# Sartor02/libMultiRobotPlanning

Hardware: AMD Instinct MI355X
Metric: low_level_node_expansions_per_sec (higher is better)
Workload: dtype int32

## Files before the change

### libmultirobotplanning_amd/csrc/ll_compact.h

```cpp
#pragma once
#include <stddef.h>
#include <stdint.h>

namespace mrp {
namespace ct {

using namespace wv;

#ifndef WV_HAS_UNMASKED_GLOADS
WV_FN V gLoadU16(const uint16_t* base, V idx) { return gLoadU16m(base, idx, bsplat(true)); }
WV_FN V gLoad32(const uint32_t* base, V idx) { return gLoad32m(base, idx, bsplat(true)); }
#endif

constexpr uint32_t kRowBytes = 128;
constexpr uint32_t oCtl = 0;
constexpr uint32_t oJob = 256;
constexpr uint32_t oRes = 384;
constexpr uint32_t oOpen = 448;
constexpr uint32_t kFront = 0xFFFFFFFFu;
template <uint32_t GROUPS, uint32_t FH_BITS, uint32_t F_BITS, uint32_t L_BITS, bool LONGT = false>
struct TierCfg {
  static constexpr bool kLongT = LONGT;
  static constexpr uint32_t kGroups = GROUPS;
  static constexpr uint32_t kCap = 256u * GROUPS - 1u;
// ... 56 lines not shown
constexpr uint32_t windowBytes(bool bg) { return Narrow::windowBytes(bg); }
constexpr uint32_t kBitsBytes = Narrow::kBitsBytes, kParentBytes = Narrow::kParentBytes;
constexpr uint32_t kMO = Narrow::kMO, kMF = Narrow::kMF, kEmpty = Narrow::kEmpty, kMaxT = Narrow::kMaxT;
constexpr uint32_t kHeapClamp = Narrow::kHeapClamp;
static_assert(oOpen % 16 == 0, "LDS areas are 16-byte aligned");

enum : int32_t { C_OK = 0, C_NO_SOLUTION = 1, C_CAP_EXP = 2, C_OVERFLOW = -1 };

struct CJob {
  uint32_t dimx, dimy, sx, sy, gx, gy;
  int32_t lastGoal;
  float w;
  uint32_t nVc, nEc;
  uint32_t obstWords;
  uint32_t nAgentsPad, tPad;
  uint32_t maxExp;
  uint32_t openCap, maxT;
  uint32_t taNoGoal;
  uint32_t rows;
  uint64_t vc;
  uint64_t ec;
  uint64_t obst;
  uint64_t pathsG;
  uint64_t parentTab;
  uint64_t outPath;
  uint64_t bitsG;
};
static_assert(sizeof(CJob) <= oRes - oJob && sizeof(CJob) % 4 == 0, "CJob fits its block of the window");
struct CRes {
  int32_t status, cost, fmin, nStates;
  uint32_t expanded, nodes;
};
#ifdef MRP_CT_PROF
#define MRP_CT_PROF_DECL uint32_t prof_[8] = {0, 0, 0, 0, 0, 0, 0, 0}; uint64_t profT_ = wv::clock64()
#define MRP_CT_PROF_MARK(k) do { const uint64_t n_ = wv::clock64(); prof_[k] += (uint32_t)(n_ - profT_); profT_ = n_; } while (0)
#define MRP_CT_PROF_ADD(k, v) prof_[k] += (v)
#define MRP_CT_PROF_STORE(lds) do { for (uint32_t q_ = 0; q_ < 8; ++q_) ldsStoreS(lds, oRes + 32u + 4u * q_, prof_[q_]); } while (0)
#elif defined(MRP_CT_ASM_MARKS)
#define MRP_CT_PROF_DECL do { } while (0)
#define MRP_CT_PROF_MARK(k) asm volatile("; PHASE " #k ::: "memory")
#define MRP_CT_PROF_ADD(k, v) do { } while (0)
#define MRP_CT_PROF_STORE(lds) do { } while (0)
#else
#define MRP_CT_PROF_DECL do { } while (0)
#define MRP_CT_PROF_MARK(k) do { } while (0)
#define MRP_CT_PROF_ADD(k, v) do { } while (0)
#define MRP_CT_PROF_STORE(lds) do { } while (0)
#endif
static_assert(sizeof(CRes) <= 32 && oRes + 64 <= oOpen, "CRes fits its block of the window");

#ifndef MRP_CT_COUNT
#define MRP_CT_COUNT(k, v) do { } while (0)
#endif

#define MRP_CT_JOB_U32(lds, field) ldsLoadS(lds, oJob + (uint32_t)offsetof(CJob, field))
template <class T>
WV_FN T* jobPtr(Lds lds, uint32_t off) {
  const uint64_t lo = ldsLoadS(lds, oJob + off), hi = ldsLoadS(lds, oJob + off + 4u);
  return (T*)(uintptr_t)(lo | (hi << 32));
}
#define MRP_CT_JOB_PTR(T, lds, field) jobPtr<T>(lds, (uint32_t)offsetof(CJob, field))

WV_FN uint32_t popc64(uint64_t v) { return (uint32_t)__builtin_popcountll(v); }
WV_FN uint32_t ctz64(uint64_t v) { return (uint32_t)__builtin_ctzll(v); }
WV_FN uint32_t ctz32(uint32_t v) { return (uint32_t)__builtin_ctz(v); }
WV_FN uint32_t lg2(uint32_t v) { return 31u - (uint32_t)__builtin_clz(v); }
WV_FN uint32_t lo32(uint64_t v) { return (uint32_t)v; }
WV_FN uint32_t hi32(uint64_t v) { return (uint32_t)(v >> 32); }

#ifndef WV_HAS_MASK_SLICES
WV_FN V maskShr(uint64_t m, V sh) { return sel((sh & 32u) != 0u, splat(hi32(m)), splat(lo32(m))) >> (sh & 16u); }
WV_FN V bitSel(V pick, V a, V b) { return (a & pick) | (b & ~pick); }
WV_FN B lowLanes(uint32_t m) { return (((splat(m) >> laneId()) & 1u) != 0u) & (laneId() < 32u); }
#endif

struct Sides {
  V lane, l5;
  B isB;
  V lvl, off1;
  V anc, needR;
};
WV_FN Sides makeSides() {
  Sides s;
  s.lane = laneId();
  s.l5 = s.lane & 31u;
  s.isB = (s.lane >> 5) != 0u;
  const V n = s.l5 + 1u;
  s.lvl = 31u - clz(n);
  s.off1 = sel(s.l5 == 31u, splat(0x100000u), n - (splat(1u) << s.lvl) - 1u);
  s.anc = splat(0u);
  s.needR = splat(0u);
  for (uint32_t k = 1; k <= 4; ++k) {
    const V a = n >> k;
    const B has = (a != 0u) & (n < 32u);
    s.anc |= sel(has, splat(1u) << (a - 1u), splat(0u));
    s.needR |= sel(has, ((n >> (k - 1u)) & 1u) << (a - 1u), splat(0u));
  }
  return s;
}
WV_FN V bothSides(const Sides& S, uint32_t a, uint32_t b) { return sel(S.isB, splat(b), splat(a)); }

WV_FN V dualDescend(Lds lds, const Sides& S, V hb, V km, V cMax, V xk) {
  V idx = splat(0u);
  for (;;) {
    const V node = ((idx + 1u) << S.lvl) + S.off1;
    V c = node * 2u + 1u;
    c = sel(c < cMax, c, cMax);
    const V2 pr = ldsLoad64(lds, hb + c * 4u);
    const V kl = pr.x & km, kr = pr.y & km;
    const B right = kl < kr;
    const V pe = sel(right, pr.y, pr.x);
    const V pk = sel(right, kr, kl);
    const B go = pk >= xk;
    const uint64_t goM = ballot(go), rM = ballot(right);
    const V g32 = bothSides(S, lo32(goM), hi32(goM));
    const V r32 = bothSides(S, lo32(rM), hi32(rM));
    const B reached = ((g32 & S.anc) == S.anc) & (((r32 ^ S.needR) & S.anc) == 0u);
    const B onPath = reached & go;
    const uint64_t pM = ballot(onPath);
    ldsStore32m(lds, hb + node * 4u, pe, onPath);
    const V pm = bothSides(S, lo32(pM), hi32(pM));
    const V steps = popc(pm);
    const V d = 31u - clz(pm | 1u);
    const V rel = d * 2u + 1u + ((r32 >> d) & 1u);
    idx = sel(pm != 0u, ((idx + 1u) << steps) + rel - (splat(1u) << steps), idx);
    if (ballot(steps == 5u) == 0ull) break;
  }
  return idx;
}

WV_FN void dualSiftUp(Lds lds, const Sides& S, V hb, V km, V p1, uint32_t e, bool idleA, bool idleB) {
  const V ancPos = (p1 >> (S.l5 + 1u)) - 1u;
  const V ae = ldsLoad32(lds, hb + ancPos * 4u);
  const uint64_t worse = ballot((ae & km) < (km & e));
  const uint32_t stopA = idleA ? 0u : ctz32(~lo32(worse)) + 1u, stopB = idleB ? 0u : ctz32(~hi32(worse)) + 1u;
  const V stop1 = bothSides(S, stopA, stopB);
  const V dest = (p1 >> S.l5) - 1u;
  ldsStore32m(lds, hb + dest * 4u, sel((S.l5 + 1u) == stop1, splat(e), ae), S.l5 < stop1);
}

struct Rows {
  V l4;
  B isY, isSecond;
};
WV_FN Rows makeRows() {
  Rows r;
  const V lane = laneId();
  r.l4 = lane & 15u;
  r.isY = (lane >> 5) != 0u;
  r.isSecond = ((lane >> 4) & 1u) != 0u;
  return r;
}
WV_FN V perRow(const Rows& R, uint32_t x1, uint32_t x2, uint32_t y1, uint32_t y2) {
  return sel(R.isY, sel(R.isSecond, splat(y2), splat(y1)), sel(R.isSecond, splat(x2), splat(x1)));
}

WV_FN void pushPairs(Lds lds, const Rows& R, uint32_t hbX, uint32_t kmX, uint32_t pX, uint32_t nX, uint32_t eX1, uint32_t eX2,
                     uint32_t hbY, uint32_t kmY, uint32_t pY, uint32_t nY, uint32_t eY1, uint32_t eY2) {
  const V hb = sel(R.isY, splat(hbY), splat(hbX));
  const V km = sel(R.isY, splat(kmY), splat(kmX));
  const V p1 = perRow(R, nX >= 1u ? pX + 1u : 1u, nX >= 2u ? pX + 2u : 1u, nY >= 1u ? pY + 1u : 1u, nY >= 2u ? pY + 2u : 1u);
  const V e = perRow(R, eX1, eX2, eY1, eY2);
  const V ek = e & km;
  const V ancIdx = p1 >> (R.l4 + 1u);
  const V ae = ldsLoad32(lds, hb + ancIdx * 4u - 4u);
  const V dest = hb + (p1 >> R.l4) * 4u - 4u;
  const uint64_t worse1 = ballot((ae & km) < ek);
  const uint32_t sX1 = nX >= 1u ? ctz32(~lo32(worse1)) + 1u : 0u, sY1 = nY >= 1u ? ctz32(~hi32(worse1)) + 1u : 0u;
  const V stop1 = sel(R.isY, splat(sY1), splat(sX1));
  ldsStore32m(lds, dest, sel((R.l4 + 1u) == stop1, e, ae), (!R.isSecond) & (R.l4 < stop1));
  if (nX >= 2u || nY >= 2u) {
#ifndef MRP_CT_PLAIN_EXPANSION
    const uint32_t ddX = ((pX + 2u) & (pX + 1u)) == 0u ? 1u : 0u, ddY = ((pY + 2u) & (pY + 1u)) == 0u ? 1u : 0u;
#else
    const uint32_t ddX = lg2(pX + 2u) - lg2(pX + 1u), ddY = lg2(pY + 2u) - lg2(pY + 1u);
#endif
    const V dd = sel(R.isY, splat(ddY), splat(ddX));
    const V e1 = sel(R.isY, splat(eY1), splat(eX1));
    const V j1p1 = R.l4 + 1u - dd;
    const B shared = (R.l4 >= dd) & (ancIdx == ((p1 - 1u) >> j1p1));
    const V up = rowShl1(ae, kFront);
    const V now = sel(shared, sel((j1p1 + 1u) < stop1, up, sel((j1p1 + 1u) == stop1, e1, ae)), sel((p1 == 2u) & (R.l4 == 0u), e1, ae));
    const uint64_t worse2 = ballot((now & km) < ek);
    const uint32_t sX2 = nX >= 2u ? ctz32(~(lo32(worse2) >> 16)) + 1u : 0u, sY2 = nY >= 2u ? ctz32(~(hi32(worse2) >> 16)) + 1u : 0u;
    const V stop2 = sel(R.isY, splat(sY2), splat(sX2));
    ldsStore32m(lds, dest, sel((R.l4 + 1u) == stop2, e, now), R.isSecond & (R.l4 < stop2));
  }
}

template <bool EPS, bool PLDS, bool BG = false, class C = Narrow>
WV_ENTRY int32_t compactSearch(Lds window) {
  constexpr uint32_t kGroups = C::kGroups, kHeapClamp = C::kHeapClamp, kAuxCap = C::kAuxCap, kAuxBytes = C::kAuxBytes,
                     kAuxClamp = C::kAuxClamp, kRows = C::kRows, kBitsBytes = C::kBitsBytes;
  constexpr uint32_t oFocal = C::oFocal, oAux = C::oAux, oBits = C::oBits;
  constexpr uint32_t kMO = C::kMO, kMF = C::kMF, kEmpty = C::kEmpty, kMOAux = C::kMOAux, kAuxShift = C::kAuxShift;
  constexpr uint32_t kFShift = C::kFShift, kFhShift = C::kFhShift, kFMax = C::kFMax, kFhMax = C::kFhMax, kGMax = C::kGMax;
  constexpr uint32_t oObstX = C::obstOff(BG), oPathsX = C::pathsOff(BG);
  constexpr uint32_t oBuild = BG ? oOpen : oBits;
  const Lds lds = windowBase(window);
  const Sides S = makeSides();
  const Rows Rw = makeRows();
  const V lane = S.lane;
  const V hb = bothSides(S, oOpen + 4u, oFocal + 4u);
  const V km = bothSides(S, kMO, kMF);
  const V hbAux = splat(oAux + 4u), kmAux = splat(kMOAux);
  const uint32_t dimx = MRP_CT_JOB_U32(lds, dimx), dimy = MRP_CT_JOB_U32(lds, dimy);
  const uint32_t gx = MRP_CT_JOB_U32(lds, gx), gy = MRP_CT_JOB_U32(lds, gy);
  const uint32_t nEc = MRP_CT_JOB_U32(lds, nEc);
  const uint32_t nAgentsPad = EPS ? MRP_CT_JOB_U32(lds, nAgentsPad) : 0u;
  int32_t status = C_NO_SOLUTION, cost = 0, fmin = 0, nStates = 0;
  uint32_t nOpen = 1, nFocal = EPS ? 1u : 0u, nodes = 1, expansions = 0;

  MRP_CT_PROF_DECL;
  sync();
  uint32_t* bitsG = BG ? MRP_CT_JOB_PTR(uint32_t, lds, bitsG) : nullptr;
  {
    const uint32_t* obst = MRP_CT_JOB_PTR(const uint32_t, lds, obst);
    const uint32_t obstWords = MRP_CT_JOB_U32(lds, obstWords);
    const V y = S.l5;
    const V bitOff = y * dimx;
    const V wi = bitOff >> 5, sh = bitOff & 31u;
    const B rowIn = (y < dimy) & !S.isB;
    const V lo = gLoad32m(obst, wi, rowIn & (wi < obstWords));
    const V hi = gLoad32m(obst, wi + 1u, rowIn & ((wi + 1u) < obstWords));
    V w = sel(sh == 0u, lo, (lo >> sh) | (hi << (splat(32u) - sh)));
    const uint32_t colMask = dimx >= 32u ? 0xFFFFFFFFu : ((1u << dimx) - 1u);
    w = (w & colMask) | ~colMask;
    w = sel(rowIn, w, splat(0xFFFFFFFFu));
    ldsStore32m(lds, splat(oObstX) + y * 4u, w, !S.isB);
  }
  auto initHeaps = [&]() {
    const V4 none{splat(kEmpty), splat(kEmpty), splat(kEmpty), splat(kEmpty)};
    const V4 head{sel(lane == 0u, splat(kFront), splat(kEmpty)), splat(kEmpty), splat(kEmpty), splat(kEmpty)};
    ldsStore128(lds, splat(oOpen) + lane * 16u, head);
    ldsStore128(lds, splat(oFocal) + lane * 16u, head);
    ldsStore128(lds, splat(oAux) + lane * 16u, head);
    for (uint32_t g = 1; g < kGroups; ++g) {
      ldsStore128(lds, splat(oOpen + g * 1024u) + lane * 16u, none);
      ldsStore128(lds, splat(oFocal + g * 1024u) + lane * 16u, none);
    }
// ... 30 lines not shown
    const V4 head{sel(lane == 0u, splat(kFront), splat(kEmpty)), splat(kEmpty), splat(kEmpty), splat(kEmpty)};
    ldsStore128(lds, splat(oAux) + lane * 16u, head);
    for (uint32_t b = 1024u; b < kAuxBytes; b += 1024u) ldsStore128m(lds, splat(oAux + b) + lane * 16u, none, (lane * 16u + b) < kAuxBytes);
    sync();
    rowsReady += kRows;
  };
  if (C::kLongT) {
    moreRows();
  } else if (BG) {
    constexpr uint32_t kBuildRows = C::kBuildRows;
    for (uint32_t r0 = 0; r0 < kRows; r0 += kBuildRows) {
      buildRows(oBuild, r0, kBuildRows);
      sync();
      for (uint32_t i = 0; i < kBuildRows * kRowBytes / 1024u; ++i)
        gStore128(bitsG, splat(r0 * (kRowBytes / 16u) + i * 64u) + lane, ldsLoad128(lds, splat(oBuild + i * 1024u) + lane * 16u));
      sync();
    }
    initHeaps();
  } else {
    buildRows(oBuild, 0u, kRows);
  }
  V ecReg = splat(0xFFFFFFFFu);
  if (nEc) {
    const uint32_t* ec = MRP_CT_JOB_PTR(const uint32_t, lds, ec);
    ldsStore32(lds, splat(oAux + 16u) + lane * 4u, sel(lane < nEc, gLoad32m(ec, lane, lane < nEc), splat(0xFFFFFFFFu)));
    sync();
    ecReg = ldsLoad32(lds, splat(oAux + 16u) + lane * 4u);
    sync();
    const V4 none{splat(kEmpty), splat(kEmpty), splat(kEmpty), splat(kEmpty)};
    ldsStore128m(lds, splat(oAux + 16u) + lane * 16u, none, lane < 16u);
  }
  const V dx = sel(lane == 1u, splat(0xFFFFFFFFu), sel(lane == 2u, splat(1u), sel(lane < 5u, splat(0u), splat(0x4000u))));
  const V dy = sel(lane == 3u, splat(1u), sel(lane == 4u, splat(0xFFFFFFFFu), splat(0u)));
#ifndef MRP_CT_PLAIN_EXPANSION
  const bool grid = EPS && nAgentsPad != 0u && nAgentsPad <= 16u;
#else
  const bool grid = false;
#endif
  const V agent0 = grid ? Rw.l4 : lane;
  const B in0 = agent0 < nAgentsPad, in1 = (lane + 64u) < nAgentsPad;
  const V col0 = sel(in0, agent0, splat(nAgentsPad ? nAgentsPad - 1u : 0u));
  const V col1 = sel(in1, lane + 64u, splat(nAgentsPad ? nAgentsPad - 1u : 0u));
  const V gridD = perRow(Rw, 0xFFFFFFFFu, 1u, 256u, 0xFFFFFF00u);
  const V gridSh = ((lane - 1u) & 3u) << 4;
  const V gridWait = sel(lane == 0u, splat(0xFFFFFFFFu), splat(0u));
  const uint32_t tPad = EPS ? MRP_CT_JOB_U32(lds, tPad) : 0u;
  const uint16_t* pathsG = PLDS ? nullptr : MRP_CT_JOB_PTR(const uint16_t, lds, pathsG);
  const int32_t lastGoal = (int32_t)MRP_CT_JOB_U32(lds, lastGoal);
  const float wBound = uintAsFloat(MRP_CT_JOB_U32(lds, w));
  const uint32_t maxExp = MRP_CT_JOB_U32(lds, maxExp), openCap = MRP_CT_JOB_U32(lds, openCap), maxT = MRP_CT_JOB_U32(lds, maxT);
  uint8_t* parentTab = MRP_CT_JOB_PTR(uint8_t, lds, parentTab);
  const uint32_t goalCell = gx | (gy << 5);
  int32_t bestF;
  {
    const uint32_t sx = MRP_CT_JOB_U32(lds, sx), sy = MRP_CT_JOB_U32(lds, sy);
    const uint32_t h0 = (sx > gx ? sx - gx : gx - sx) + (sy > gy ? sy - gy : gy - sy);
    bestF = (int32_t)h0;
    const uint32_t e0 = (kFhMax << kFhShift) | ((kFMax - h0) << kFShift) | ((C::kLongT ? 63u - h0 : 0u) << 10) | (sx | (sy << 5));
    ldsStoreS(lds, oOpen + 4u, e0);
    if (EPS) ldsStoreS(lds, oFocal + 4u, e0);
  }
  sync();
  MRP_CT_PROF_MARK(0);

  for (;;) {
    if (nOpen == 0u) {
      status = C_NO_SOLUTION;
      break;
    }
    const V tops = ldsLoad32(lds, hb);
    const uint32_t topO = readlane(tops, 0);
    uint32_t curE = EPS ? readlane(tops, 32) : topO;
    if (EPS) {
      const int32_t fTop = (int32_t)(kFMax - ((topO >> kFShift) & kFMax));
      const int32_t oldBest = bestF;
      bestF = fTop;
      if (fTop > oldBest) {
        MRP_CT_PROF_MARK(0);
        const float lo = fmulRn((float)oldBest, wBound), hi = fmulRn((float)fTop, wBound);
        bool bandEmpty = false;
#ifndef MRP_CT_FORCE_WALK
        {
          const int32_t fA = (int32_t)lo + 1, fBraw = (int32_t)hi;
          const int32_t fB = fBraw > (int32_t)kFMax - 1 ? (int32_t)kFMax - 1 : fBraw;
          bandEmpty = true;
          if (fB >= fA) {
            const V base = splat(kFMax - (uint32_t)fB), span = splat((uint32_t)(fB - fA));
            for (uint32_t g = 0; g < kGroups && g * 256u <= nOpen; ++g) {
              const V4 grp = ldsLoad128(lds, splat(oOpen + g * 1024u) + lane * 16u);
              const B in = ((((grp.x >> kFShift) & kFMax) - base) <= span) | ((((grp.y >> kFShift) & kFMax) - base) <= span) |
                           ((((grp.z >> kFShift) & kFMax) - base) <= span) | ((((grp.w >> kFShift) & kFMax) - base) <= span);
              if (ballot(in)) {
                bandEmpty = false;
                break;
              }
            }
          }
        }
#endif
        MRP_CT_PROF_ADD(7, bandEmpty ? 1u : 0u);
        if (!bandEmpty) {
        uint32_t npq = 0, npqHigh = 0;
        uint32_t cur = 0, curKey = topO & kMO, eCur = topO;
        V trio = ldsLoad32(lds, splat(oOpen + 4u) + sel(lane == 2u, splat(cur), splat(2u * cur + 1u) + (lane & 1u)) * 4u);
        for (;;) {
          MRP_CT_PROF_ADD(6, 1u);
          const uint32_t firstC = 2u * cur + 1u;
          const uint32_t nCh = firstC + 1u < nOpen ? 2u : firstC < nOpen ? 1u : 0u;
          if (npq + 2u > kAuxCap) {
            status = C_OVERFLOW;
            cost = 4;
            break;
          }
          const uint32_t e1 = readlane(trio, 0), e2 = readlane(trio, 1);
          const float fv = (float)(int32_t)(kFMax - ((curKey >> kFShift) & kFMax));
          const bool inBand = fv > lo && fv <= hi;
          pushPairs(lds, Rw, oAux + 4u, kMOAux, npq, nCh, ((e1 & kMO) << kAuxShift) | firstC, ((e2 & kMO) << kAuxShift) | (firstC + 1u),
                    oFocal + 4u, kMF, nFocal,
                    inBand ? 1u : 0u, eCur, 0u);
          npq += nCh;
          nFocal += inBand ? 1u : 0u;
          npqHigh = npq > npqHigh ? npq : npqHigh;
          if (fv > hi) break;
          if (npq == 0u) break;
          npq -= 1u;
          const V two = ldsLoad32(lds, splat(oAux + 4u) + sel(lane == 0u, splat(0u), splat(npq)) * 4u);
          ldsStoreS(lds, oAux + 4u + 4u * npq, kEmpty);
          uint32_t hole = 0, above = kFront;
          bool first = true;
          uint32_t value = 0;
          for (;;) {
            const V node = ((splat(hole) + 1u) << S.lvl) + S.off1;
            V c = node * 2u + 1u;
            c = sel(c < kAuxClamp, c, splat(kAuxClamp));
            const V2 pr = ldsLoad64(lds, splat(oAux + 4u) + c * 4u);
            if (first) {
              first = false;
              const uint32_t curA = readlane(two, 0);
              value = readlane(two, 1);
              cur = curA & C::kAuxIdxMask;
              curKey = (curA >> kAuxShift) & kMO;
              trio = ldsLoad32(lds, splat(oOpen + 4u) + sel(lane == 2u, splat(cur), splat(2u * cur + 1u) + (lane & 1u)) * 4u);
              if (npq == 0u) break;
            }
            const V kl = pr.x & kMOAux, kr = pr.y & kMOAux;
            const B right = kr >= kl;
            const V pe = sel(right, pr.y, pr.x);
            const B go = kl > (kEmpty & kMOAux);
            const uint32_t goM = lo32(ballot(go)), rM = lo32(ballot(right));
            const B onPath = ((S.anc & goM) == S.anc) & (((S.needR ^ rM) & S.anc) == 0u) & go;
            const uint32_t pm = lo32(ballot(onPath & !S.isB));
            ldsStore32m(lds, splat(oAux + 4u) + node * 4u, pe, onPath);
            if (pm == 0u) break;
            const uint32_t steps = (uint32_t)__builtin_popcount(pm), d = lg2(pm);
            hole = ((hole + 1u) << steps) + 2u * d + 1u + ((rM >> d) & 1u) - (1u << steps);
            above = readlane(pe, d);
            if (steps < 5u) break;
          }
          eCur = readlane(trio, 2);
          if (npq > 0u) {
            if (hole == 0u || !((above & kMOAux) < (value & kMOAux)))
              ldsStoreS(lds, oAux + 4u + 4u * hole, value);
            else
              dualSiftUp(lds, S, hbAux, kmAux, splat(hole + 1u), value, false, false);
          }
        }
        for (uint32_t b = 0; b <= 4u * npqHigh; b += 1024u) {
          const V4 none{splat(kEmpty), splat(kEmpty), splat(kEmpty), splat(kEmpty)};
          const V4 head{sel(lane == 0u, splat(kFront), splat(kEmpty)), splat(kEmpty), splat(kEmpty), splat(kEmpty)};
          ldsStore128m(lds, splat(oAux + b) + lane * 16u, b == 0u ? head : none, (lane * 16u + b) < kAuxBytes);
        }
        if (status == C_OVERFLOW) break;
        curE = ldsLoadS(lds, oFocal + 4u);
        }
        MRP_CT_PROF_MARK(1);
      }
    }
    const uint32_t cell = curE & 1023u, curFh = kFhMax - (curE >> kFhShift);
    const uint32_t t = C::kLongT ? (kFMax - ((curE >> kFShift) & kFMax)) - (63u - ((curE >> 10) & 63u)) : (curE >> 10) & kGMax;
    const uint32_t x = cell & 31u, y = cell >> 5;
    const bool isGoal = cell == goalCell && (int32_t)t > lastGoal;
    if (!isGoal) {
      if (nOpen + 5u > openCap || t > maxT || (EPS && !C::kExactFhCheck && curFh + 2u * nAgentsPad > kFhMax)) {
        status = C_OVERFLOW;
        cost = nOpen + 5u > openCap ? 1 : t > maxT ? 2 : 3;
        break;
      }
    }
    expansions += 1u;
    if (expansions > maxExp) {
      status = C_CAP_EXP;
      break;
    }
    if (isGoal) {
      status = C_OK;
      cost = (int32_t)t;
      fmin = (int32_t)(kFMax - (((EPS ? topO : curE) >> kFShift) & kFMax));
      nStates = (int32_t)t + 1;
      uint16_t* outPath = MRP_CT_JOB_PTR(uint16_t, lds, outPath);
      sync();
      uint32_t c = cell;
      const uint32_t* tab32 = (const uint32_t*)parentTab;
      constexpr int32_t kStage = BG ? (int32_t)C::kStageRows : 8;
      for (int32_t k0 = (int32_t)t; k0 >= 1; k0 -= kStage) {
        V rowW[kStage][4];
        for (int32_t r = 0; r < kStage; ++r)
          for (uint32_t q = 0; q < 4; ++q)
            rowW[r][q] = (k0 - r >= 1) ? gLoad32Coherent(tab32, splat((uint32_t)(k0 - r) * 256u + q * 64u) + lane) : splat(0u);
        for (int32_t r = 0; r < kStage; ++r)
          for (uint32_t q = 0; q < 4; ++q) ldsStore32(lds, splat(oBuild + (uint32_t)r * 1024u + q * 256u) + lane * 4u, rowW[r][q]);
        sync();
        for (int32_t r = 0; r < kStage && k0 - r >= 1; ++r) {
          const uint32_t k = (uint32_t)(k0 - r);
          gStoreU16m(outPath, splat(k), splat((c & 31u) | ((c >> 5) << 8)), lane == 0u);
          const uint32_t a = first(ldsLoadU8(lds, splat(oBuild + (uint32_t)r * 1024u + c)));
          c = a == 1u ? c + 1u : a == 2u ? c - 1u : a == 3u ? c - 32u : a == 4u ? c + 32u : c;
        }
        sync();
      }
      gStoreU16m(outPath, splat(0u), splat((c & 31u) | ((c >> 5) << 8)), lane == 0u);
      break;
    }

    MRP_CT_PROF_MARK(0);
    const uint32_t t1 = t + 1u;
    if (C::kLongT && t1 >= rowsReady) moreRows();
// ... 21 lines not shown
          a1 = gLoadU16(pathsG, splat(ra * nAgentsPad) + col1);
          b1 = gLoadU16(pathsG, splat(rb * nAgentsPad) + col1);
        }
      }
    }

    MRP_CT_PROF_MARK(2);
    {
      const uint32_t nOld = nOpen;
      nOpen -= 1u;
      if (EPS) nFocal -= 1u;
      const V lastAddr = hb + bothSides(S, nOpen, nFocal) * 4u;
      const V lastV = ldsLoad32(lds, lastAddr);
      uint32_t p = 0;
#ifndef MRP_CT_PLAIN_EXPANSION
      const bool atRoot = EPS && ((curE ^ topO) & C::kStateMask) == 0u;
#else
      const bool atRoot = false;
#endif
      MRP_CT_COUNT(0, atRoot ? 1u : 0u);
      MRP_CT_COUNT(6, atRoot && nOld > 512u ? 1u : 0u);
      if (EPS && !atRoot) {
        const V key = splat(curE & C::kStateMask);
        for (uint32_t g = 0; g < kGroups && g * 256u <= nOld; ++g) {
          MRP_CT_COUNT(1, 1u);
          const V4 grp = ldsLoad128(lds, splat(oOpen + g * 1024u) + lane * 16u);
          const B m0 = (grp.x & C::kStateMask) == key, m1 = (grp.y & C::kStateMask) == key, m2 = (grp.z & C::kStateMask) == key,
                  m3 = (grp.w & C::kStateMask) == key;
          const uint64_t any = ballot(m0 | m1 | m2 | m3);
          if (any) {
            const V pos = lane * 4u + sel(m0, splat(0xFFFFFFFFu), sel(m1, splat(0u), sel(m2, splat(1u), splat(2u))));
            p = g * 256u + readlane(pos, ctz64(any));
            if (kGroups > 4u) break;
          }
        }
      }
      uint32_t lastO = readlane(lastV, 0);
      const uint32_t lastF = EPS ? readlane(lastV, 32) : kFront;
      ldsStore32m(lds, lastAddr, splat(kEmpty), S.l5 == 0u);
      if (EPS && !atRoot) {
        const uint32_t depth = lg2(p + 1u);
        MRP_CT_COUNT(4, p >= 256u ? 1u : 0u);
        MRP_CT_COUNT(5, p == nOld - 1u && depth != 0u ? 1u : 0u);
        const B act = !S.isB & (S.l5 < depth);
        const V ancPos = (splat(p + 1u) >> (S.l5 + 1u)) - 1u;
        const V ae = ldsLoad32(lds, splat(oOpen + 4u) + ancPos * 4u);
        ldsStore32m(lds, splat(oOpen + 4u) + ((splat(p + 1u) >> S.l5) - 1u) * 4u, ae, act);
        if (p == nOld - 1u && depth != 0u) {
          lastO = readlane(ae, 0);
          ldsStoreS(lds, oOpen + 4u + 4u * p, kEmpty);
        }
      }
      const V xk = bothSides(S, lastO & kMO, lastF & kMF);
      const V hole = dualDescend(lds, S, hb, km, splat(kHeapClamp), xk);
      ldsStore32m(lds, hb + hole * 4u, bothSides(S, lastO, lastF), (S.l5 == 0u) & (bothSides(S, nOpen, EPS ? nFocal : 0u) != 0u));
    }

    MRP_CT_PROF_MARK(3);
    const B okV = inb & (((word >> (nx & 31u)) & 1u) == 0u);
    uint32_t mask = lo32(ballot(okV)) & 0x1Fu;
    if (nEc) {
      const uint32_t base = (t << 19) | ((y * dimx + x) << 3);
      const V d = ecReg - base;
      if (ballot(d < 5u)) {
        uint32_t blocked = 0;
        for (uint32_t k = 0; k < 5u; ++k) blocked |= ballot(d == k) ? (1u << k) : 0u;
        mask &= ~blocked;
      }
    }
    if (mask == 0u) {
      MRP_CT_PROF_MARK(4);
      continue;
    }

#ifndef MRP_CT_PLAIN_EXPANSION
    const B mine = lowLanes(mask);
#else
    const B mine = (lane < 5u) & (((splat(mask) >> lane) & 1u) != 0u);
#endif
    const V f = sad(nx, splat(gx), sad(ny, splat(gy), splat(t1)));
    V fhV = splat(curFh);
    if (EPS && nAgentsPad) {
      const uint32_t curXy = x | (y << 8);
      const uint64_t valid0 = PLDS ? ~0ull : ballot(in0);
      const uint64_t swap0 = ballot(b0 == curXy) & valid0;
      if (grid) {
        MRP_CT_COUNT(2, 1u);
        const V gcell = splat(curXy) + gridD;
        const uint64_t vM = ballot(b0 == gcell) & valid0, sM = ballot(a0 == gcell) & swap0;
        const uint64_t sWait = ballot(a0 == curXy) & swap0;
        const V ofRows = (maskShr(vM, gridSh) & 0xFFFFu) | (maskShr(sM, gridSh) << 16);
        const uint32_t ofWait = (lo32(swap0) & 0xFFFFu) | (lo32(sWait) << 16);
        fhV = splat(curFh) + popc(bitSel(gridWait, splat(ofWait), ofRows));
      } else {
        MRP_CT_COUNT(3, 1u);
        const V nxy = nx | (ny << 8);
        const uint64_t valid1 = PLDS ? ~0ull : nAgentsPad > 64u ? ballot(in1) : 0ull;
        const uint64_t swap1 = nAgentsPad > 64u ? ballot(b1 == curXy) & valid1 : 0ull;
        for (uint32_t mm = mask; mm; mm &= mm - 1u) {
          const uint32_t k = ctz32(mm);
          const uint32_t cc = readlane(nxy, k);
          uint32_t cnt = popc64(ballot(b0 == cc) & valid0) + popc64(ballot(a0 == cc) & swap0);
          if (nAgentsPad > 64u) cnt += popc64(ballot(b1 == cc) & valid1) + popc64(ballot(a1 == cc) & swap1);
          fhV = writelane(fhV, curFh + cnt, k);
        }
      }
    }
    if (EPS && C::kExactFhCheck && ballot(mine & (fhV > kFhMax))) {
      status = C_OVERFLOW;
      cost = 3;
      break;
    }
    const V lowKey = C::kLongT ? (splat(63u + t1) - f) << 10 : splat(t1 << 10);
    const V eV = ((splat(kFhMax) - fhV) << kFhShift) | ((splat(kFMax) - f) << kFShift) | lowKey | ncell;
    uint32_t maskF = 0;
    if (EPS) {
      const float bound = fmulRn((float)bestF, wBound);
      maskF = lo32(ballot(mine & leF32(cvtF32(f), bound)));
    }
    if (BG) {
#ifndef MRP_CT_PLAIN_EXPANSION
      const uint32_t rowBits = (uint32_t)(((uint64_t)((0x75643120u >> ((mask & 7u) << 2)) & 7u) << x) >> 1);
#else
      const uint32_t bx = 1u << x;
      const uint32_t rowBits = ((mask & 1u) ? bx : 0u) | ((mask & 2u) ? bx >> 1 : 0u) | ((mask & 4u) ? bx << 1 : 0u);
#endif
      gStore32and8m(bitsG, wordIdx, word | sel(lane < 3u, splat(rowBits), splat(1u) << (nx & 31u)), parentTab,
                    splat(t1 << 10) + ncell, lane, mine);
    } else {
      ldsOr32m(lds, wordAddr, splat(1u) << (nx & 31u), mine);
      gStore8m(parentTab, splat(t1 << 10) + ncell, lane, mine);
    }
    nodes += (uint32_t)__builtin_popcount(mask);
    MRP_CT_PROF_MARK(4);
    for (uint32_t mm = mask; mm;) {
      const uint32_t k1 = ctz32(mm);
      mm &= mm - 1u;
      const bool two = mm != 0u;
      const uint32_t k2 = two ? ctz32(mm) : 0u;
      mm &= mm - 1u;
      const uint32_t e1 = readlane(eV, k1), e2 = readlane(eV, k2);
      const bool f1 = EPS && ((maskF >> k1) & 1u), f2 = EPS && two && ((maskF >> k2) & 1u);
      const uint32_t nX = two ? 2u : 1u, nY = (f1 ? 1u : 0u) + (f2 ? 1u : 0u);
#ifndef MRP_CT_NO_SINGLE_PUSH
      if (!two)
        dualSiftUp(lds, S, hb, km, bothSides(S, nOpen + 1u, f1 ? nFocal + 1u : 1u), e1, false, !f1);
      else
#endif
        pushPairs(lds, Rw, oOpen + 4u, kMO, nOpen, nX, e1, e2, oFocal + 4u, kMF, nFocal, nY, f1 ? e1 : e2, e2);
      nOpen += nX;
      nFocal += nY;
    }
    MRP_CT_PROF_MARK(5);
  }
  ldsStoreS(lds, oRes + (uint32_t)offsetof(CRes, status), (uint32_t)status);
  ldsStoreS(lds, oRes + (uint32_t)offsetof(CRes, cost), (uint32_t)cost);
  ldsStoreS(lds, oRes + (uint32_t)offsetof(CRes, fmin), (uint32_t)fmin);
  ldsStoreS(lds, oRes + (uint32_t)offsetof(CRes, nStates), (uint32_t)nStates);
  ldsStoreS(lds, oRes + (uint32_t)offsetof(CRes, expanded), expansions);
  ldsStoreS(lds, oRes + (uint32_t)offsetof(CRes, nodes), nodes);
  MRP_CT_PROF_STORE(lds);
  sync();
  return status;
}

constexpr uint32_t kTaKm = 0x7FFF0000u;
enum : int32_t { C_CAP_NODES = 3, C_CAP_HORIZON = 4 };
WV_ENTRY int32_t compactSearchTA(Lds window) {
  const Lds lds = windowBase(window);
  const Sides S = makeSides();
  const V lane = S.lane;
  const V hbO = splat(oOpen + 4u), kmO = splat(kTaKm);
  const uint32_t dimx = MRP_CT_JOB_U32(lds, dimx), dimy = MRP_CT_JOB_U32(lds, dimy);
  const uint32_t gx = MRP_CT_JOB_U32(lds, gx), gy = MRP_CT_JOB_U32(lds, gy);
  const uint32_t nEc = MRP_CT_JOB_U32(lds, nEc), nVc = MRP_CT_JOB_U32(lds, nVc);
  const bool noGoal = MRP_CT_JOB_U32(lds, taNoGoal) != 0u;
  int32_t status = C_NO_SOLUTION, cost = 0, fmin = 0, nStates = 0;
  uint32_t nOpen = 1, nodes = 1, expansions = 0;
  sync();
  {
    const uint32_t* obst = MRP_CT_JOB_PTR(const uint32_t, lds, obst);
    const uint32_t obstWords = MRP_CT_JOB_U32(lds, obstWords);
    const V y = S.l5;
    const V bitOff = y * dimx;
    const V wi = bitOff >> 5, sh = bitOff & 31u;
    const B rowIn = (y < dimy) & !S.isB;
    const V lo = gLoad32m(obst, wi, rowIn & (wi < obstWords));
    const V hi = gLoad32m(obst, wi + 1u, rowIn & ((wi + 1u) < obstWords));
    V w = sel(sh == 0u, lo, (lo >> sh) | (hi << (splat(32u) - sh)));
    const uint32_t colMask = dimx >= 32u ? 0xFFFFFFFFu : ((1u << dimx) - 1u);
    w = (w & colMask) | ~colMask;
    w = sel(rowIn, w, splat(0xFFFFFFFFu));
    ldsStore32m(lds, splat(oObst) + y * 4u, w, !S.isB);
  }
  {
    const V4 none{splat(kEmpty), splat(kEmpty), splat(kEmpty), splat(kEmpty)};
    const V4 head{sel(lane == 0u, splat(kFront), splat(kEmpty)), splat(kEmpty), splat(kEmpty), splat(kEmpty)};
    const V4 zero{splat(0u), splat(0u), splat(0u), splat(0u)};
    ldsStore128(lds, splat(oOpen) + lane * 16u, head);
    for (uint32_t g = 1; g < kGroups; ++g) ldsStore128(lds, splat(oOpen + g * 1024u) + lane * 16u, none);
    ldsStore128m(lds, splat(oOpen + kGroups * 1024u), none, lane == 0u);
    for (uint32_t i = 0; i < kRows / 8u; ++i) ldsStore128(lds, splat(oBits + i * 1024u) + lane * 16u, zero);
    if (!noGoal) {
      const uint32_t* heur = (const uint32_t*)MRP_CT_JOB_PTR(const uint16_t, lds, pathsG);
      for (uint32_t q = 0; q < 8u; ++q) ldsStore32(lds, splat(oPaths + q * 256u) + lane * 4u, gLoad32m(heur, splat(q * 64u) + lane, bsplat(true)));
// ... 159 lines not shown
```

### libmultirobotplanning_amd/csrc/wave_dev.h

```cpp
#pragma once
#ifdef MRP_WV_BOOL_PREDICATES
#include "wave_dev_bool.h"
#else
#include <hip/hip_runtime.h>
#include <stdint.h>

namespace wv {

#define WV_FN __device__ __forceinline__
#define WV_ENTRY __device__ __attribute__((noinline))

struct V {
  uint32_t v;
  WV_FN V() {}
  WV_FN V(uint32_t s) : v(s) {}
};
struct B {
  uint64_t m;
};
typedef uint32_t v4u __attribute__((ext_vector_type(4)));
typedef uint32_t v2u __attribute__((ext_vector_type(2)));
struct V2 { V x, y; };
struct V4 { V x, y, z, w; };
#define WV_BIN(op) WV_FN V operator op(V a, V b) { return V(a.v op b.v); }
// ... 13 lines not shown
#define WV_CMP(op) WV_FN B operator op(V a, V b) { return B{__builtin_amdgcn_ballot_w64(a.v op b.v)}; }
WV_CMP(<)
WV_CMP(<=)
WV_CMP(>)
WV_CMP(>=)
WV_CMP(==)
WV_CMP(!=)
#undef WV_CMP
WV_FN B operator&(B a, B b) { return B{a.m & b.m}; }
WV_FN B operator|(B a, B b) { return B{a.m | b.m}; }
WV_FN B operator!(B a) { return B{~a.m}; }
WV_FN bool lanePred(B b) { return __builtin_amdgcn_inverse_ballot_w64(b.m); }

typedef __attribute__((address_space(3))) uint8_t* Lds;

WV_FN Lds windowBase(Lds) { return (Lds)(uintptr_t)0; }
WV_FN V laneId() { return V(threadIdx.x); }
WV_FN uint64_t clock64() { return __builtin_amdgcn_s_memtime(); }
WV_FN V splat(uint32_t s) { return V(s); }
WV_FN V sel(B c, V a, V b) { return V(lanePred(c) ? a.v : b.v); }
WV_FN B bsplat(bool s) { return B{s ? ~0ull : 0ull}; }
WV_FN uint64_t ballot(B p) { return p.m; }
WV_FN uint32_t readlane(V v, uint32_t lane) { return __builtin_amdgcn_readlane(v.v, lane); }
WV_FN uint32_t first(V v) { return __builtin_amdgcn_readfirstlane(v.v); }
extern "C" __device__ int mrp_llvm_writelane(int val, int lane, int old) __asm("llvm.amdgcn.writelane.i32");
WV_FN V writelane(V v, uint32_t val, uint32_t lane) { return V((uint32_t)mrp_llvm_writelane((int)val, (int)lane, (int)v.v)); }
WV_FN V shr1(V v) { return V((uint32_t)__builtin_amdgcn_update_dpp((int)v.v, (int)v.v, 0x138, 0xF, 0xF, false)); }
WV_FN V rowShl1(V v, uint32_t fill) { return V((uint32_t)__builtin_amdgcn_update_dpp((int)fill, (int)v.v, 0x101, 0xF, 0xF, false)); }
WV_FN V bpermute(V v, V src) { return V((uint32_t)__builtin_amdgcn_ds_bpermute((int)((src.v & 63u) << 2), (int)v.v)); }
WV_FN B laneMask(uint64_t m) { return B{m}; }
#define WV_HAS_MASK_SLICES 1
WV_FN V maskShr(uint64_t m, V sh) { return V((uint32_t)(m >> (sh.v & 63u))); }
WV_FN V bitSel(V pick, V a, V b) { return V((a.v & pick.v) | (b.v & ~pick.v)); }
WV_FN B lowLanes(uint32_t m) { return B{(uint64_t)m}; }
WV_FN uint32_t waveMinU32(V v) {
  uint32_t x = v.v;
#define WV_MIN_STEP(ctrl)                                                                              \
  {                                                                                                    \
    const uint32_t t = (uint32_t)__builtin_amdgcn_update_dpp((int)0xFFFFFFFFu, (int)x, ctrl, 0xF, 0xF, false); \
    x = t < x ? t : x;                                                                                 \
  }
  WV_MIN_STEP(0x111)
  WV_MIN_STEP(0x112)
  WV_MIN_STEP(0x114)
  WV_MIN_STEP(0x118)
#undef WV_MIN_STEP
  const uint32_t a = __builtin_amdgcn_readlane(x, 15), b = __builtin_amdgcn_readlane(x, 31);
  const uint32_t c = __builtin_amdgcn_readlane(x, 47), d = __builtin_amdgcn_readlane(x, 63);
  const uint32_t ab = a < b ? a : b, cd = c < d ? c : d;
  return ab < cd ? ab : cd;
}
WV_FN V clz(V v) { return V((uint32_t)__builtin_clz(v.v)); }
WV_FN V popc(V v) { return V((uint32_t)__builtin_popcount(v.v)); }
WV_FN float uintAsFloat(uint32_t v) { return __uint_as_float(v); }
WV_FN V sad(V a, V b, V c) { return V(((a.v > b.v ? a.v : b.v) - (a.v > b.v ? b.v : a.v)) + c.v); }
WV_FN float fmulRn(float a, float b) { return __fmul_rn(a, b); }
WV_FN V cvtF32(V v) { return V(__float_as_uint((float)v.v)); }
WV_FN B leF32(V aBits, float b) { return B{__builtin_amdgcn_ballot_w64(__uint_as_float(aBits.v) <= b)}; }

WV_FN V ldsLoad32(Lds l, V addr) { return V(*(__attribute__((address_space(3))) uint32_t*)(l + addr.v)); }
WV_FN V ldsLoad32m(Lds l, V addr, B m) { return V(lanePred(m) ? *(__attribute__((address_space(3))) uint32_t*)(l + addr.v) : 0u); }
WV_FN V ldsLoadU16(Lds l, V addr) { return V(*(__attribute__((address_space(3))) uint16_t*)(l + addr.v)); }
WV_FN V ldsLoadU8(Lds l, V addr) { return V(*(__attribute__((address_space(3))) uint8_t*)(l + addr.v)); }
WV_FN V2 ldsLoad64m(Lds l, V addr, B m) {
  V2 r{V(0u), V(0u)};
  if (lanePred(m)) {
    const v2u t = *(__attribute__((address_space(3))) v2u*)(l + addr.v);
    r.x = V(t.x);
    r.y = V(t.y);
  }
  return r;
}
WV_FN V2 ldsLoad64(Lds l, V addr) {
  const v2u t = *(__attribute__((address_space(3))) v2u*)(l + addr.v);
  return V2{V(t.x), V(t.y)};
}
WV_FN V4 ldsLoad128(Lds l, V addr) {
  const v4u t = *(__attribute__((address_space(3))) v4u*)(l + addr.v);
  return V4{V(t.x), V(t.y), V(t.z), V(t.w)};
}
WV_FN void ldsStore32m(Lds l, V addr, V val, B m) {
  if (lanePred(m)) *(__attribute__((address_space(3))) uint32_t*)(l + addr.v) = val.v;
}
WV_FN void ldsStore32(Lds l, V addr, V val) { *(__attribute__((address_space(3))) uint32_t*)(l + addr.v) = val.v; }
WV_FN void ldsStore128(Lds l, V addr, V4 val) {
  v4u t;
  t.x = val.x.v; t.y = val.y.v; t.z = val.z.v; t.w = val.w.v;
  *(__attribute__((address_space(3))) v4u*)(l + addr.v) = t;
}
WV_FN void ldsStore128m(Lds l, V addr, V4 val, B m) {
  if (lanePred(m)) ldsStore128(l, addr, val);
}
WV_FN void ldsStore8m(Lds l, V addr, V val, B m) {
  if (lanePred(m)) *(__attribute__((address_space(3))) uint8_t*)(l + addr.v) = (uint8_t)val.v;
}
WV_FN void ldsStoreU16m(Lds l, V addr, V val, B m) {
  if (lanePred(m)) *(__attribute__((address_space(3))) uint16_t*)(l + addr.v) = (uint16_t)val.v;
}
WV_FN void ldsOr32m(Lds l, V addr, V bits, B m) {
  if (lanePred(m))
    __hip_atomic_fetch_or((__attribute__((address_space(3))) uint32_t*)(l + addr.v), bits.v, __ATOMIC_RELAXED,
                          __HIP_MEMORY_SCOPE_WORKGROUP);
}
WV_FN uint32_t ldsLoadS(Lds l, uint32_t addr) { return __builtin_amdgcn_readfirstlane(*(__attribute__((address_space(3))) uint32_t*)(l + addr)); }
WV_FN void ldsStoreS(Lds l, uint32_t addr, uint32_t val) { *(__attribute__((address_space(3))) uint32_t*)(l + addr) = val; }

// ... 41 lines not shown
```

### libmultirobotplanning_amd/csrc/wave_dev_bool.h

```cpp
#pragma once
#include <hip/hip_runtime.h>
#include <stdint.h>

namespace wv {

#define WV_FN __device__ __forceinline__
#define WV_ENTRY __device__ __attribute__((noinline))

typedef uint32_t V;
typedef bool B;
typedef uint32_t v4u __attribute__((ext_vector_type(4)));
typedef uint32_t v2u __attribute__((ext_vector_type(2)));
struct V2 { V x, y; };
struct V4 { V x, y, z, w; };

typedef __attribute__((address_space(3))) uint8_t* Lds;

WV_FN Lds windowBase(Lds) { return (Lds)(uintptr_t)0; }
WV_FN V laneId() { return threadIdx.x; }
WV_FN uint64_t clock64() { return __builtin_amdgcn_s_memtime(); }
WV_FN V splat(uint32_t s) { return s; }
WV_FN V sel(B c, V a, V b) { return c ? a : b; }
WV_FN B bsplat(bool s) { return s; }
WV_FN uint64_t ballot(B p) { return __builtin_amdgcn_ballot_w64(p); }
WV_FN uint32_t readlane(V v, uint32_t lane) { return __builtin_amdgcn_readlane(v, lane); }
WV_FN uint32_t first(V v) { return __builtin_amdgcn_readfirstlane(v); }
extern "C" __device__ int mrp_llvm_writelane(int val, int lane, int old) __asm("llvm.amdgcn.writelane.i32");
WV_FN V writelane(V v, uint32_t val, uint32_t lane) { return (uint32_t)mrp_llvm_writelane((int)val, (int)lane, (int)v); }
WV_FN B laneMask(uint64_t m) { return ((m >> threadIdx.x) & 1u) != 0u; }
WV_FN uint32_t waveMinU32(V v) {
  uint32_t x = v;
#define WV_MIN_STEP(ctrl)                                                                              \
  {                                                                                                    \
    const uint32_t t = (uint32_t)__builtin_amdgcn_update_dpp((int)0xFFFFFFFFu, (int)x, ctrl, 0xF, 0xF, false); \
    x = t < x ? t : x;                                                                                 \
  }
  WV_MIN_STEP(0x111)
  WV_MIN_STEP(0x112)
  WV_MIN_STEP(0x114)
  WV_MIN_STEP(0x118)
#undef WV_MIN_STEP
  const uint32_t a = __builtin_amdgcn_readlane(x, 15), b = __builtin_amdgcn_readlane(x, 31);
  const uint32_t c = __builtin_amdgcn_readlane(x, 47), d = __builtin_amdgcn_readlane(x, 63);
  const uint32_t ab = a < b ? a : b, cd = c < d ? c : d;
  return ab < cd ? ab : cd;
}
WV_FN V shr1(V v) { return (uint32_t)__builtin_amdgcn_update_dpp((int)v, (int)v, 0x138, 0xF, 0xF, false); }
WV_FN V rowShl1(V v, uint32_t fill) { return (uint32_t)__builtin_amdgcn_update_dpp((int)fill, (int)v, 0x101, 0xF, 0xF, false); }
WV_FN V clz(V v) { return (uint32_t)__builtin_clz(v); }
WV_FN V popc(V v) { return (uint32_t)__builtin_popcount(v); }
WV_FN float uintAsFloat(uint32_t v) { return __uint_as_float(v); }
WV_FN V sad(V a, V b, V c) { return ((a > b ? a : b) - (a > b ? b : a)) + c; }
WV_FN float fmulRn(float a, float b) { return __fmul_rn(a, b); }
WV_FN V cvtF32(V v) { return __float_as_uint((float)v); }
WV_FN B leF32(V aBits, float b) { return __uint_as_float(aBits) <= b; }

WV_FN V ldsLoad32(Lds l, V addr) { return *(__attribute__((address_space(3))) uint32_t*)(l + addr); }
WV_FN V ldsLoad32m(Lds l, V addr, B m) { return m ? *(__attribute__((address_space(3))) uint32_t*)(l + addr) : 0u; }
WV_FN V ldsLoadU16(Lds l, V addr) { return *(__attribute__((address_space(3))) uint16_t*)(l + addr); }
WV_FN V ldsLoadU8(Lds l, V addr) { return *(__attribute__((address_space(3))) uint8_t*)(l + addr); }
WV_FN V2 ldsLoad64m(Lds l, V addr, B m) {
  V2 r{0u, 0u};
  if (m) {
    const v2u t = *(__attribute__((address_space(3))) v2u*)(l + addr);
    r.x = t.x;
    r.y = t.y;
  }
  return r;
}
WV_FN V2 ldsLoad64(Lds l, V addr) {
  const v2u t = *(__attribute__((address_space(3))) v2u*)(l + addr);
  return V2{t.x, t.y};
}
WV_FN V4 ldsLoad128(Lds l, V addr) {
  const v4u t = *(__attribute__((address_space(3))) v4u*)(l + addr);
  return V4{t.x, t.y, t.z, t.w};
}
WV_FN void ldsStore32m(Lds l, V addr, V val, B m) {
  if (m) *(__attribute__((address_space(3))) uint32_t*)(l + addr) = val;
}
WV_FN void ldsStore32(Lds l, V addr, V val) { *(__attribute__((address_space(3))) uint32_t*)(l + addr) = val; }
WV_FN void ldsStore128(Lds l, V addr, V4 val) {
  v4u t;
  t.x = val.x; t.y = val.y; t.z = val.z; t.w = val.w;
  *(__attribute__((address_space(3))) v4u*)(l + addr) = t;
}
WV_FN void ldsStore128m(Lds l, V addr, V4 val, B m) {
  if (m) ldsStore128(l, addr, val);
}
WV_FN V bpermute(V v, V src) { return (uint32_t)__builtin_amdgcn_ds_bpermute((int)((src & 63u) << 2), (int)v); }
WV_FN void ldsStoreU16m(Lds l, V addr, V val, B m) {
  if (m) *(__attribute__((address_space(3))) uint16_t*)(l + addr) = (uint16_t)val;
}
WV_FN void ldsStore8m(Lds l, V addr, V val, B m) {
  if (m) *(__attribute__((address_space(3))) uint8_t*)(l + addr) = (uint8_t)val;
}
WV_FN void ldsOr32m(Lds l, V addr, V bits, B m) {
  if (m)
    __hip_atomic_fetch_or((__attribute__((address_space(3))) uint32_t*)(l + addr), bits, __ATOMIC_RELAXED,
                          __HIP_MEMORY_SCOPE_WORKGROUP);
}
WV_FN uint32_t ldsLoadS(Lds l, uint32_t addr) { return first(*(__attribute__((address_space(3))) uint32_t*)(l + addr)); }
WV_FN void ldsStoreS(Lds l, uint32_t addr, uint32_t val) { *(__attribute__((address_space(3))) uint32_t*)(l + addr) = val; }
// ... 41 lines not shown
```

Baseline: 1.398 billion.

## Vectorize paired heap pushes per turn and add optional kept-heap-root tracking

```diff
diff --git a/libmultirobotplanning_amd/csrc/ll_compact.h b/libmultirobotplanning_amd/csrc/ll_compact.h
--- a/libmultirobotplanning_amd/csrc/ll_compact.h
+++ b/libmultirobotplanning_amd/csrc/ll_compact.h
@@ -132,6 +132,10 @@
 #ifndef MRP_CT_COUNT
 #define MRP_CT_COUNT(k, v) do { } while (0)
 #endif
+#ifndef MRP_CT_COUNT_SLOTS
+#define MRP_CT_COUNT_SLOTS 7
+#endif
+#define MRP_CT_COUNTX(k, v) do { if ((k) < MRP_CT_COUNT_SLOTS) MRP_CT_COUNT(k, v); } while (0)
 
 #define MRP_CT_JOB_U32(lds, field) ldsLoadS(lds, oJob + (uint32_t)offsetof(CJob, field))
 template <class T>
@@ -147,6 +151,30 @@
 WV_FN uint32_t lg2(uint32_t v) { return 31u - (uint32_t)__builtin_clz(v); }
 WV_FN uint32_t lo32(uint64_t v) { return (uint32_t)v; }
 WV_FN uint32_t hi32(uint64_t v) { return (uint32_t)(v >> 32); }
+
+#ifndef WV_HAS_CTZ
+WV_FN V ctz(V v) { return splat(31u) - clz(v & (splat(0u) - v)); }
+#endif
+
+#ifdef MRP_CT_PLAIN_EXPANSION
+#ifndef MRP_CT_SCALAR_PUSHES
+#define MRP_CT_SCALAR_PUSHES
+#endif
+#ifndef MRP_CT_LOAD_TOPS
+#define MRP_CT_LOAD_TOPS
+#endif
+#endif
+#if !defined(MRP_CT_LOAD_TOPS) && !defined(MRP_CT_KEEP_TOPS) && !defined(MRP_CT_CHECK_TOPS)
+#define MRP_CT_LOAD_TOPS
+#endif
+#ifdef MRP_CT_LOAD_TOPS
+#define MRP_CT_KEPT_TOPS false
+#else
+#define MRP_CT_KEPT_TOPS true
+#endif
+#if defined(MRP_CT_CHECK_TOPS) && (defined(MRP_CT_LOAD_TOPS) || defined(__HIP_DEVICE_COMPILE__))
+#error "MRP_CT_CHECK_TOPS checks the kept heap roots: an emulator build without MRP_CT_LOAD_TOPS"
+#endif
 
 #ifndef WV_HAS_MASK_SLICES
 WV_FN V maskShr(uint64_t m, V sh) { return sel((sh & 32u) != 0u, splat(hi32(m)), splat(lo32(m))) >> (sh & 16u); }
@@ -180,7 +208,8 @@
 }
 WV_FN V bothSides(const Sides& S, uint32_t a, uint32_t b) { return sel(S.isB, splat(b), splat(a)); }
 
-WV_FN V dualDescend(Lds lds, const Sides& S, V hb, V km, V cMax, V xk) {
+template <bool TOP>
+WV_FN V dualDescendT(Lds lds, const Sides& S, V hb, V km, V cMax, V xk, V& top) {
   V idx = splat(0u);
   for (;;) {
     const V node = ((idx + 1u) << S.lvl) + S.off1;
@@ -192,6 +221,7 @@
     const V pe = sel(right, pr.y, pr.x);
     const V pk = sel(right, kr, kl);
     const B go = pk >= xk;
+    if (TOP) top = sel(go & (node == 0u), pe, top);
     const uint64_t goM = ballot(go), rM = ballot(right);
     const V g32 = bothSides(S, lo32(goM), hi32(goM));
     const V r32 = bothSides(S, lo32(rM), hi32(rM));
@@ -208,6 +238,10 @@
   }
   return idx;
 }
+WV_FN V dualDescend(Lds lds, const Sides& S, V hb, V km, V cMax, V xk) {
+  V none = splat(0u);
+  return dualDescendT<false>(lds, S, hb, km, cMax, xk, none);
+}
 
 WV_FN void dualSiftUp(Lds lds, const Sides& S, V hb, V km, V p1, uint32_t e, bool idleA, bool idleB) {
   const V ancPos = (p1 >> (S.l5 + 1u)) - 1u;
@@ -222,6 +256,7 @@
 struct Rows {
   V l4;
   B isY, isSecond;
+  V rowSh, heapSh;
 };
 WV_FN Rows makeRows() {
   Rows r;
@@ -229,6 +264,8 @@
   r.l4 = lane & 15u;
   r.isY = (lane >> 5) != 0u;
   r.isSecond = ((lane >> 4) & 1u) != 0u;
+  r.rowSh = lane & 48u;
+  r.heapSh = lane & 32u;
   return r;
 }
 WV_FN V perRow(const Rows& R, uint32_t x1, uint32_t x2, uint32_t y1, uint32_t y2) {
@@ -266,6 +303,37 @@
     const V stop2 = sel(R.isY, splat(sY2), splat(sX2));
     ldsStore32m(lds, dest, sel((R.l4 + 1u) == stop2, e, now), R.isSecond & (R.l4 < stop2));
   }
+}
+
+WV_FN V rowStop(uint64_t worse, V rowSh) { return ctz(~maskShr(worse, rowSh)) + 1u; }
+
+template <bool TOPS>
+WV_FN void pushTurn(Lds lds, const Rows& R, V hb, V km, V sideBits, uint32_t pair, uint32_t low, uint32_t e1s, uint32_t e2s, V& n,
+                    V& tops) {
+  const V pf = sideBits & pair;
+  const V cnt = popc(pf);
+  const B act = sel(R.isSecond, cnt >> 1u, cnt) != 0u;
+  const V p1 = sel(act, sel(R.isSecond, n + 2u, n + 1u), splat(1u));
+  const V e1 = sel((pf & low) != 0u, splat(e1s), splat(e2s));
+  const V e = sel(R.isSecond, splat(e2s), e1);
+  const V ek = e & km;
+  const V ancIdx = p1 >> (R.l4 + 1u);
+  const V ae = ldsLoad32(lds, hb + ancIdx * 4u - 4u);
+  const V dest = hb + (p1 >> R.l4) * 4u - 4u;
+  const V stop1 = rowStop(ballot((ae & km) < ek), R.heapSh);
+  ldsStore32m(lds, dest, sel((R.l4 + 1u) == stop1, e, ae), (!R.isSecond) & act & (R.l4 < stop1));
+  if (TOPS) tops = sel(((tops & km) < (e1 & km)) & (cnt != 0u), e1, tops);
+  if ((pair ^ low) != 0u) {
+    const V dd = sel((p1 & (p1 - 1u)) == 0u, splat(1u), splat(0u));
+    const V j1p1 = R.l4 + 1u - dd;
+    const B shared = (R.l4 >= dd) & (ancIdx == ((p1 - 1u) >> j1p1));
+    const V up = rowShl1(ae, kFront);
+    const V now = sel(shared, sel((j1p1 + 1u) < stop1, up, sel((j1p1 + 1u) == stop1, e1, ae)), sel((p1 == 2u) & (R.l4 == 0u), e1, ae));
+    const V stop2 = rowStop(ballot((now & km) < ek), R.rowSh);
+    ldsStore32m(lds, dest, sel((R.l4 + 1u) == stop2, e, now), R.isSecond & act & (R.l4 < stop2));
+    if (TOPS) tops = sel(((tops & km) < (splat(e2s) & km)) & (cnt > 1u), splat(e2s), tops);
+  }
+  n += cnt;
 }
 
 template <bool EPS, bool PLDS, bool BG = false, class C = Narrow>
@@ -402,6 +470,7 @@
   uint8_t* parentTab = MRP_CT_JOB_PTR(uint8_t, lds, parentTab);
   const uint32_t goalCell = gx | (gy << 5);
   int32_t bestF;
+  V tops;
   {
     const uint32_t sx = MRP_CT_JOB_U32(lds, sx), sy = MRP_CT_JOB_U32(lds, sy);
     const uint32_t h0 = (sx > gx ? sx - gx : gx - sx) + (sy > gy ? sy - gy : gy - sy);
@@ -409,6 +478,7 @@
     const uint32_t e0 = (kFhMax << kFhShift) | ((kFMax - h0) << kFShift) | ((C::kLongT ? 63u - h0 : 0u) << 10) | (sx | (sy << 5));
     ldsStoreS(lds, oOpen + 4u, e0);
     if (EPS) ldsStoreS(lds, oFocal + 4u, e0);
+    tops = splat(e0);
   }
   sync();
   MRP_CT_PROF_MARK(0);
@@ -418,7 +488,15 @@
       status = C_NO_SOLUTION;
       break;
     }
-    const V tops = ldsLoad32(lds, hb);
+#ifdef MRP_CT_LOAD_TOPS
+    tops = ldsLoad32(lds, hb);
+#elif defined(MRP_CT_CHECK_TOPS)
+    {
+      const V seen = ldsLoad32(lds, hb);
+      MRP_CT_COUNTX(8, 1u);
+      MRP_CT_COUNTX(9, (readlane(seen, 0) != readlane(tops, 0) || (EPS && readlane(seen, 32) != readlane(tops, 32))) ? 1u : 0u);
+    }
+#endif
     const uint32_t topO = readlane(tops, 0);
     uint32_t curE = EPS ? readlane(tops, 32) : topO;
     if (EPS) {
@@ -522,6 +600,9 @@
         }
         if (status == C_OVERFLOW) break;
         curE = ldsLoadS(lds, oFocal + 4u);
+#ifndef MRP_CT_LOAD_TOPS
+        tops = sel(S.isB, splat(curE), tops);
+#endif
         }
         MRP_CT_PROF_MARK(1);
       }
@@ -649,8 +730,21 @@
         }
       }
       const V xk = bothSides(S, lastO & kMO, lastF & kMF);
+      const V x = bothSides(S, lastO, lastF);
+      const B some = bothSides(S, nOpen, EPS ? nFocal : 0u) != 0u;
+#ifdef MRP_CT_LOAD_TOPS
       const V hole = dualDescend(lds, S, hb, km, splat(kHeapClamp), xk);
-      ldsStore32m(lds, hb + hole * 4u, bothSides(S, lastO, lastF), (S.l5 == 0u) & (bothSides(S, nOpen, EPS ? nFocal : 0u) != 0u));
+#else
+      V top = x;
+      const V hole = dualDescendT<true>(lds, S, hb, km, splat(kHeapClamp), xk, top);
+      MRP_CT_COUNTX(10, nOpen != 0u && readlane(top, 0) == lastO ? 1u : 0u);
+      MRP_CT_COUNTX(11, nOpen != 0u && readlane(top, 0) != lastO ? 1u : 0u);
+      MRP_CT_COUNTX(12, EPS && nFocal != 0u && readlane(top, 32) == lastF ? 1u : 0u);
+      MRP_CT_COUNTX(13, EPS && nFocal != 0u && readlane(top, 32) != lastF ? 1u : 0u);
+      tops = sel(some, top, splat(kEmpty));
+#endif
+      MRP_CT_COUNTX(7, EPS && !atRoot ? 1u : 0u);
+      ldsStore32m(lds, hb + hole * 4u, x, (S.l5 == 0u) & some);
     }
 
     MRP_CT_PROF_MARK(3);
@@ -730,6 +824,47 @@
     }
     nodes += (uint32_t)__builtin_popcount(mask);
     MRP_CT_PROF_MARK(4);
+#ifndef MRP_CT_SCALAR_PUSHES
+    {
+      const V sideBits = bothSides(S, mask, maskF);
+      V nV = bothSides(S, nOpen, nFocal);
+      const uint32_t nSucc = (uint32_t)__builtin_popcount(mask);
+      MRP_CT_COUNTX(16, nSucc == 3u ? 1u : 0u);
+      MRP_CT_COUNTX(17, nSucc == 4u ? 1u : 0u);
+      MRP_CT_COUNTX(18, nSucc == 5u ? 1u : 0u);
+      for (uint32_t mm = mask; mm;) {
+        const uint32_t rest1 = mm & (mm - 1u);
+        const uint32_t rest2 = rest1 & (rest1 - 1u);
+        const uint32_t low = mm ^ rest1, pair = mm ^ rest2;
+        const uint32_t e1 = readlane(eV, ctz32(mm)), e2 = readlane(eV, ctz32(rest1 | 32u));
+        if (MRP_CT_COUNT_SLOTS > 14) {
+          const bool two = rest1 != 0u, f1 = (maskF & low) != 0u, f2 = (maskF & pair & ~low) != 0u;
+          const uint32_t pO = readlane(nV, 0), pF = readlane(nV, 32), rO = readlane(tops, 0), rF = readlane(tops, 32);
+          MRP_CT_COUNTX(14, two ? 0u : 1u);
+          MRP_CT_COUNTX(15, two ? 1u : 0u);
+          MRP_CT_COUNTX(19, f1 != f2 ? 1u : 0u);
+          MRP_CT_COUNTX(20, f1 && f2 ? 1u : 0u);
+          MRP_CT_COUNTX(21, !f1 && f2 ? 1u : 0u);
+          MRP_CT_COUNTX(22, two && ((pO + 2u) & (pO + 1u)) == 0u ? 1u : 0u);
+          MRP_CT_COUNTX(23, f1 && f2 && ((pF + 2u) & (pF + 1u)) == 0u ? 1u : 0u);
+          MRP_CT_COUNTX(24, (pO == 0u ? 1u : 0u) + ((f1 || f2) && pF == 0u ? 1u : 0u));
+          const uint32_t eF1 = f1 ? e1 : e2;
+          const bool o1 = pO == 0u || (rO & kMO) < (e1 & kMO), fr1 = (f1 || f2) && (pF == 0u || (rF & kMF) < (eF1 & kMF));
+          MRP_CT_COUNTX(25, o1 ? 1u : 0u);
+          MRP_CT_COUNTX(26, fr1 ? 1u : 0u);
+          MRP_CT_COUNTX(27, two && o1 && (e1 & kMO) < (e2 & kMO) ? 1u : 0u);
+          MRP_CT_COUNTX(28, f1 && f2 && fr1 && (e1 & kMF) < (e2 & kMF) ? 1u : 0u);
+          const uint32_t rO2 = o1 ? e1 : rO, rF2 = fr1 ? eF1 : rF;
+          MRP_CT_COUNTX(29, (pO != 0u && (rO & kMO) == (e1 & kMO) ? 1u : 0u) + (two && (rO2 & kMO) == (e2 & kMO) ? 1u : 0u));
+          MRP_CT_COUNTX(30, ((f1 || f2) && pF != 0u && (rF & kMF) == (eF1 & kMF) ? 1u : 0u) + (f1 && f2 && (rF2 & kMF) == (e2 & kMF) ? 1u : 0u));
+        }
+        pushTurn<MRP_CT_KEPT_TOPS>(lds, Rw, hb, km, sideBits, pair, low, e1, e2, nV, tops);
+        mm = rest2;
+      }
+      nOpen += nSucc;
+      nFocal += (uint32_t)__builtin_popcount(maskF);
+    }
+#else
     for (uint32_t mm = mask; mm;) {
       const uint32_t k1 = ctz32(mm);
       mm &= mm - 1u;
@@ -745,9 +880,17 @@
       else
 #endif
         pushPairs(lds, Rw, oOpen + 4u, kMO, nOpen, nX, e1, e2, oFocal + 4u, kMF, nFocal, nY, f1 ? e1 : e2, e2);
+#ifndef MRP_CT_LOAD_TOPS
+      {
+        const V cntS = bothSides(S, nX, nY), first = bothSides(S, e1, f1 ? e1 : e2);
+        tops = sel(((tops & km) < (first & km)) & (cntS != 0u), first, tops);
+        tops = sel(((tops & km) < (splat(e2) & km)) & (cntS > 1u), splat(e2), tops);
+      }
+#endif
       nOpen += nX;
       nFocal += nY;
     }
+#endif
     MRP_CT_PROF_MARK(5);
   }
   ldsStoreS(lds, oRes + (uint32_t)offsetof(CRes, status), (uint32_t)status);
diff --git a/libmultirobotplanning_amd/csrc/wave_dev.h b/libmultirobotplanning_amd/csrc/wave_dev.h
--- a/libmultirobotplanning_amd/csrc/wave_dev.h
+++ b/libmultirobotplanning_amd/csrc/wave_dev.h
@@ -89,6 +89,8 @@
 }
 WV_FN V clz(V v) { return V((uint32_t)__builtin_clz(v.v)); }
 WV_FN V popc(V v) { return V((uint32_t)__builtin_popcount(v.v)); }
+#define WV_HAS_CTZ 1
+WV_FN V ctz(V v) { return V((uint32_t)__builtin_ctz(v.v)); }
 WV_FN float uintAsFloat(uint32_t v) { return __uint_as_float(v); }
 WV_FN V sad(V a, V b, V c) { return V(((a.v > b.v ? a.v : b.v) - (a.v > b.v ? b.v : a.v)) + c.v); }
 WV_FN float fmulRn(float a, float b) { return __fmul_rn(a, b); }
diff --git a/libmultirobotplanning_amd/csrc/wave_dev_bool.h b/libmultirobotplanning_amd/csrc/wave_dev_bool.h
--- a/libmultirobotplanning_amd/csrc/wave_dev_bool.h
+++ b/libmultirobotplanning_amd/csrc/wave_dev_bool.h
@@ -49,6 +49,8 @@
 WV_FN V rowShl1(V v, uint32_t fill) { return (uint32_t)__builtin_amdgcn_update_dpp((int)fill, (int)v, 0x101, 0xF, 0xF, false); }
 WV_FN V clz(V v) { return (uint32_t)__builtin_clz(v); }
 WV_FN V popc(V v) { return (uint32_t)__builtin_popcount(v); }
+#define WV_HAS_CTZ 1
+WV_FN V ctz(V v) { return (uint32_t)__builtin_ctz(v); }
 WV_FN float uintAsFloat(uint32_t v) { return __uint_as_float(v); }
 WV_FN V sad(V a, V b, V c) { return ((a > b ? a : b) - (a > b ? b : a)) + c; }
 WV_FN float fmulRn(float a, float b) { return __fmul_rn(a, b); }
```

Result: faster. 1.496 billion, median of 6 (+7.0%).
